# AIM-Harvard/pyradiomics

Measured on AMD Instinct MI355X. Metric: Mvoxels/s for GLCM+GLRLM build, 512^3 vol @32 bins, higher is better.
Workload: dtype u8 levels / u32 counts / f64 out; 1 GPU; GLCM+GLRLM matrix build, 512^3 int32+uint8 volume resident in HBM, 32 grey levels, full mask, 13 angles, uniform levels; one volume per GPU (batch sharding, no collective); size=512, levels=32, dist=uniform, deferred_mode=pipeline

## Files before the change

### pyradiomics_amd/csrc/kernels_sweepfw.h

```cpp
#pragma once
#include "kernels_sweep.h"

namespace prad {

enum FwPhase { FP_INIT, FP_GRAB, FP_CTRL, FP_ISSUE, FP_WAIT_ROWS, FP_WAIT_PACK, FP_GROUP, FP_PACK, FP_SLOW, FP_FLUSH, FP_DRAIN,
               FP_TOTAL, FP_REALTIME, FP_NGROUP, FP_NGROUP_PACK, FP_NSLOW, FP_COUNT };
#ifdef PRAD_FW_STAMPS
__device__ unsigned long long prad_fw_stamps[2 * 8192 * FP_COUNT];
struct FwClock {
  unsigned long long last, first, rt0;
  unsigned acc[FP_COUNT];
  __device__ __forceinline__ void start() {
#pragma unroll
    for (int i = 0; i < FP_COUNT; i++) acc[i] = 0;
    rt0 = __builtin_amdgcn_s_memrealtime();
    first = last = __builtin_readcyclecounter();
  }
  template <int PH>
  __device__ __forceinline__ void lap() {
    const unsigned long long now = __builtin_readcyclecounter();
    acc[PH] += (unsigned)(now - last);
    last = now;
  }
  template <int PH>
  __device__ __forceinline__ void count() { acc[PH]++; }
  __device__ __forceinline__ void store(int slot) {
    acc[FP_TOTAL] = (unsigned)(__builtin_readcyclecounter() - first);
    acc[FP_REALTIME] = (unsigned)(__builtin_amdgcn_s_memrealtime() - rt0);
    const unsigned w = blockIdx.x * (blockDim.x >> 6) + (threadIdx.x >> 6);
    if ((threadIdx.x & 63) == 0 && w < 8192) {
#pragma unroll
      for (int i = 0; i < FP_COUNT; i++) prad_fw_stamps[((size_t)slot * 8192 + w) * FP_COUNT + i] = acc[i];
    }
  }
};
#else
struct FwClock {
  __device__ __forceinline__ void start() {}
  template <int PH>
  __device__ __forceinline__ void lap() {}
  template <int PH>
  __device__ __forceinline__ void count() {}
  __device__ __forceinline__ void store(int) {}
};
#endif

struct FwDesc {
  int slot;
  int NM, NU;
  int du, dx;
  long long sM, sU;
  int CL, pieces;
  int chunks;
  int dom_kind;
};
struct FwSet {
  int count;
  int NX;
  int pitch;
  int nrows;
  int xcd;
  int first_block[PRAD_MAX_SWEEP + 1];
  FwDesc d[PRAD_MAX_SWEEP];
};

struct PackJob {
  const int *image;
  const uint8_t *mask;
  uint8_t *levels;
  uint8_t *levels16;
  uint8_t *rowzero;
  int *flags;
  long long n16;
  int NX, Ng;
  int every;
};

#define PRAD_FW_U 8
#ifndef PRAD_FW_MAXG
#define PRAD_FW_MAXG 4
#endif
#define PRAD_FW_WORK_STRIDE 64
#define PRAD_FW_DOMAINS 8
__host__ __device__ inline size_t fw_lds_bytes(const HistLayout &h) { return 4 * ((size_t)h.words + (size_t)(h.Ng + 1)); }


struct FwTab {
  u32 *rl_long;
  int Nr, P4, Q, lenlim, gB, RL4, RS, RL, dummy0b, alive0, deadmax;
  unsigned Qinv;
  __device__ __forceinline__ void init(const HistLayout &h, int Nr_, u32 *rl_long_) {
    rl_long = rl_long_;
    Nr = Nr_;
    Q = 4 * (h.Ng + 1);
    P4 = (h.RS + 1) * (h.Ng + 1);
    lenlim = (h.RS + 1) * Q;
    RS = h.RS;
    RL = h.RL;
    RL4 = 4 * h.RL;
    gB = Q + 4 * h.g0 - RL4 - 4 * h.RS;
    Qinv = (unsigned)((0x100000000ull + (unsigned)Q - 1) / (unsigned)Q);
    dummy0b = Q + 4 * h.dummy0;
    alive0 = (h.RS + 2) * Q;
    deadmax = (h.RS + 1) * Q;
  }
};

__device__ __noinline__ void fw_long_event(const FwTab &T, int lv, int lb) {
  const int idx = (int)__umulhi((unsigned)lb, T.Qinv);
  if (idx < T.RS + T.RL) {
    lds_bump(T.gB + __mul24(lv, T.RL4) + (idx << 2));
    return;
  }
  const unsigned key = ((unsigned)lv << 20) | (unsigned)idx;
  bool pending = true;
// ... 650 lines not shown
          row -= du * NU;
          off -= (long long)du * NU * D.sU;
          ri -= (long long)du * NU * sUr;
          zpos = 65;
          wrap = false;
          continue;
        }
        t++;
        zpos++;
        row += du;
        off += delta;
        ri += dri;
        if (du != 0 && (row < 0 || row >= NU)) wrap = true;
      }
    }
  }
};

template <bool ZA>
__device__ __forceinline__ void fw_row_word(const FwTab &T, u32 one, int &s, u32 c, u32 x) {
  int t;
#define PRAD_FW_RCOL(J)                                                                                          \
  "v_cmpx_ne_u32_sdwa vcc, %[c], %[x] src0_sel:BYTE_" #J " src1_sel:BYTE_" #J "\n\t"                             \
  "v_add_u32_sdwa %[t], %[s], %[c] dst_sel:DWORD dst_unused:UNUSED_PAD src0_sel:DWORD src1_sel:BYTE_" #J "\n\t"   \
  "v_mul_u32_u24_sdwa %[s], %[P4], %[c] dst_sel:DWORD dst_unused:UNUSED_PAD src0_sel:DWORD src1_sel:BYTE_" #J "\n\t" \
  "v_cmpx_ne_u32_sdwa vcc, %[x], %[z] src0_sel:BYTE_" #J " src1_sel:DWORD\n\t"                                  \
  "ds_add_u32 %[t], %[one]\n\t"                                                                                  \
  "s_mov_b64 exec, -1\n\t"                                                                                       \
  "v_add_u32 %[s], %[Q], %[s]\n\t"
#define PRAD_FW_RCOL_NZ(J)                                                                                       \
  "v_cmpx_ne_u32_sdwa vcc, %[c], %[x] src0_sel:BYTE_" #J " src1_sel:BYTE_" #J "\n\t"                             \
  "v_add_u32_sdwa %[t], %[s], %[c] dst_sel:DWORD dst_unused:UNUSED_PAD src0_sel:DWORD src1_sel:BYTE_" #J "\n\t"   \
  "ds_add_u32 %[t], %[one]\n\t"                                                                                  \
  "v_mul_u32_u24_sdwa %[s], %[P4], %[c] dst_sel:DWORD dst_unused:UNUSED_PAD src0_sel:DWORD src1_sel:BYTE_" #J "\n\t" \
  "s_mov_b64 exec, -1\n\t"                                                                                       \
  "v_add_u32 %[s], %[Q], %[s]\n\t"
  if (ZA) {
    u32 z = 0;
    asm volatile("" : "+v"(z));
    asm volatile(PRAD_FW_RCOL(0) PRAD_FW_RCOL(1) PRAD_FW_RCOL(2) PRAD_FW_RCOL(3)
                 : [s] "+v"(s), [t] "=&v"(t)
                 : [c] "v"(c), [x] "v"(x), [one] "v"(one), [P4] "s"(T.P4), [Q] "s"(T.Q), [z] "v"(z)
                 : "vcc", "memory");
  } else {
    asm volatile(PRAD_FW_RCOL_NZ(0) PRAD_FW_RCOL_NZ(1) PRAD_FW_RCOL_NZ(2) PRAD_FW_RCOL_NZ(3)
                 : [s] "+v"(s), [t] "=&v"(t)
                 : [c] "v"(c), [x] "v"(x), [one] "v"(one), [P4] "s"(T.P4), [Q] "s"(T.Q)
                 : "vcc", "memory");
  }
#undef PRAD_FW_RCOL
#undef PRAD_FW_RCOL_NZ
}

template <bool LONG, bool ZA>
__device__ __forceinline__ void fw_rows_role(const HistLayout &h, const FwTab &T, u32 *lds, const uint8_t *__restrict__ L,
                                             long long nrows, int NX, int pitch, int bx, int nblocks) {
  const int lane = threadIdx.x & 63, wave = threadIdx.x >> 6, wpb = blockDim.x >> 6;
  const int dummy = T.dummy0b + 4 * lane;
  u32 one = 1;
  asm volatile("" : "+v"(one));
  uint8_t *tile = reinterpret_cast<uint8_t *>(lds) + ((fw_lds_bytes(h) + 15) & ~(size_t)15) + (size_t)wave * 64 * PRAD_ROW_PITCH;
  const int RSTEP = nrows >= 4096 ? 8 : 1;
  const long long ngroups = RSTEP == 8 ? ((nrows + 511) / 512) * 8 : (nrows + 63) / 64;
  const long long nwaves = (long long)nblocks * wpb;
  const bool vec16 = (pitch & 15) == 0 && ((uintptr_t)L & 15) == 0;
  for (long long grp = (long long)bx * wpb + wave; grp < ngroups; grp += nwaves) {
    const long long r0 = RSTEP == 8 ? (grp >> 3) * 512 + (grp & 7) : grp * 64;
    int s = 0;
    u32 pw = 0;
    uint4 nx4[4];
    auto fetch = [&](int xc) __attribute__((always_inline)) {
#pragma unroll
      for (int j = 0; j < 4; j++) {
        const int rr = j * 16 + (lane >> 2);
        const int cx = xc + (lane & 3) * 16;
        uint4 q = make_uint4(0, 0, 0, 0);
        if (r0 + RSTEP * rr < nrows && cx < NX) {
          q = *reinterpret_cast<const uint4 *>(L + (r0 + RSTEP * rr) * pitch + cx);
          const int valid = NX - cx;
          if (valid < 16) {
            u32 *qw = reinterpret_cast<u32 *>(&q);
#pragma unroll
            for (int wd = 0; wd < 4; wd++) {
              const int keep = valid - 4 * wd;
              qw[wd] = keep >= 4 ? qw[wd] : (keep <= 0 ? 0u : (qw[wd] & ((1u << (8 * keep)) - 1u)));
            }
          }
        }
        nx4[j] = q;
      }
    };
    if (vec16) fetch(0);
    for (int xc = 0; xc < NX; xc += 64) {
      if (vec16) {
#pragma unroll
        for (int j = 0; j < 4; j++) *reinterpret_cast<uint4 *>(tile + (j * 16 + (lane >> 2)) * PRAD_ROW_PITCH + (lane & 3) * 16) = nx4[j];
        __builtin_amdgcn_wave_barrier();
        if (xc + 64 < NX) fetch(xc + 64);
      } else {
        const bool xin = xc + lane < NX;
#pragma unroll 8
        for (int rr = 0; rr < 64; rr++) {
          uint8_t b = 0;
          if (xin && r0 + RSTEP * rr < nrows) b = L[(r0 + RSTEP * rr) * pitch + xc + lane];
          tile[rr * PRAD_ROW_PITCH + lane] = b;
        }
      }
      __builtin_amdgcn_wave_barrier();
      const uint4 *row = reinterpret_cast<const uint4 *>(tile + lane * PRAD_ROW_PITCH);
#pragma unroll
      for (int q = 0; q < 4; q++) {
        const uint4 d = row[q];
        const u32 wds[4] = {d.x, d.y, d.z, d.w};
        const unsigned m = (pw >> 24) ? (unsigned)(s - __mul24((int)(pw >> 24), T.P4)) : 0u;
        if (LONG && __ballot(m + 16 * T.Q > (unsigned)T.lenlim) != 0) {
#pragma unroll 1
          for (int k = 0; k < 4; k++) {
            const u32 c = wds[k], x = __builtin_amdgcn_alignbyte(c, pw, 3);
            const unsigned m4 = (pw >> 24) ? (unsigned)(s - __mul24((int)(pw >> 24), T.P4)) : 0u;
            if (__ballot(m4 + 4 * T.Q > (unsigned)T.lenlim) != 0) {
#pragma unroll
              for (int b = 0; b < 4; b++) fw_checked<LONG>(T, dummy, s, (int)((x >> (8 * b)) & 0xffu), (int)((c >> (8 * b)) & 0xffu), false);
            } else {
              fw_row_word<ZA>(T, one, s, c, x);
            }
            pw = c;
          }
        } else {
#pragma unroll
          for (int k = 0; k < 4; k++) {
            fw_row_word<ZA>(T, one, s, wds[k], __builtin_amdgcn_alignbyte(wds[k], pw, 3));
            pw = wds[k];
          }
        }
      }
      __builtin_amdgcn_wave_barrier();
    }
    fw_checked<LONG>(T, dummy, s, (int)(pw >> 24), 0, false);
  }
}

template <bool LONG>
__global__ void __launch_bounds__(1024) sweep_fw_rows_kernel(const uint8_t *__restrict__ L, long long nrows, int NX, int pitch,
                                                            int slot, int Ng, int Nr, int RS, u32 *__restrict__ glcm_acc,
                                                            u32 *__restrict__ glrlm_acc, int *__restrict__ flags) {
  extern __shared__ u32 lds[];
  if (flags[0]) return;
  const HistLayout h = hist_layout(true, true, true, Ng, RS);
  if ((unsigned)(size_t)((lds_u32 *)lds) != 0u) {
    if (threadIdx.x == 0) atomicExch(flags + 2, 1);
    return;
  }
  for (int i = threadIdx.x; i < h.words + Ng + 1; i += blockDim.x) lds[i] = 0;
  __syncthreads();
  FwTab T;
  T.init(h, Nr, glrlm_acc + (size_t)slot * Ng * Nr);
  if (flags[3] != 0) fw_rows_role<LONG, true>(h, T, lds, L, nrows, NX, pitch, (int)blockIdx.x, (int)gridDim.x);
  else fw_rows_role<LONG, false>(h, T, lds, L, nrows, NX, pitch, (int)blockIdx.x, (int)gridDim.x);
  flush_block_hist<true, true, true>(lds + Ng + 1, h, Nr, slot, glcm_acc, glrlm_acc);
}

template <bool LONG, int K, bool HASPAD, bool PACK>
__global__ void __launch_bounds__(1024) sweep_fw_kernel(FwSet set, PackJob pj, const uint8_t *__restrict__ L,
                                                        const uint8_t *__restrict__ rowzero, int Ng, int Nr, int RS,
                                                        u32 *__restrict__ glcm_acc, u32 *__restrict__ glrlm_acc,
                                                        int *__restrict__ work, int *__restrict__ flags) {
  extern __shared__ u32 lds[];
  int role = 0;
  while (role + 1 < set.count && (int)blockIdx.x >= set.first_block[role + 1]) role++;
  const int bx = (int)blockIdx.x - set.first_block[role], nblocks = set.first_block[role + 1] - set.first_block[role];
  const int wpb = (int)(blockDim.x >> 6);
  const long long pw = __builtin_amdgcn_readfirstlane((int)(blockIdx.x * wpb + (threadIdx.x >> 6)));
  PackWave pk(pj, pw, (long long)gridDim.x * wpb);
  FwClock clk;
  clk.start();
#ifdef PRAD_FW_SETPRIO
  __builtin_amdgcn_s_setprio(PRAD_FW_SETPRIO);
#endif
  if (flags[0] == 0) {
    const bool anyzero = flags[3] != 0;
    const HistLayout h = hist_layout(true, true, true, Ng, RS);
    if ((unsigned)(size_t)((lds_u32 *)lds) != 0u) {
      if (threadIdx.x == 0) atomicExch(flags + 2, 1);
    } else {
      for (int i = threadIdx.x; i < h.words + Ng + 1; i += blockDim.x) lds[i] = 0;
      __syncthreads();
      clk.lap<FP_INIT>();
      const FwDesc &D = set.d[role];
      FwTab T;
      T.init(h, Nr, glrlm_acc + (size_t)D.slot * Ng * Nr);
      int *wk = work + PRAD_FW_WORK_STRIDE * PRAD_FW_DOMAINS * role;
      if (D.dx == 0) {
        FwWave<LONG, K, 0, HASPAD, PACK> w(T, set.NX);
        w.run(D, set.NX, set.pitch, set.nrows, L, rowzero, anyzero, wk, bx, nblocks, pk, pj, set.xcd != 0, clk);
      } else if (D.dx > 0) {
        FwWave<LONG, K, 1, HASPAD, PACK> w(T, set.NX);
        w.run(D, set.NX, set.pitch, set.nrows, L, rowzero, anyzero, wk, bx, nblocks, pk, pj, set.xcd != 0, clk);
      } else {
        FwWave<LONG, K, -1, HASPAD, PACK> w(T, set.NX);
        w.run(D, set.NX, set.pitch, set.nrows, L, rowzero, anyzero, wk, bx, nblocks, pk, pj, set.xcd != 0, clk);
      }
      clk.lap<FP_CTRL>();
      flush_block_hist<true, true, true>(lds + Ng + 1, h, Nr, D.slot, glcm_acc, glrlm_acc);
      clk.lap<FP_FLUSH>();
    }
  }
  if (PACK) pk.drain(pj);
  clk.lap<FP_DRAIN>();
  clk.store(PACK ? 1 : 0);
}

}
```

### pyradiomics_amd/csrc/prad_api.hip

```cpp
#include "prad_runtime.h"
#include "kernels_generic.h"
#include "kernels_pairs.h"
#include "kernels_sweep.h"
#include "kernels_sweepfw.h"
#include "kernels_sweepfw2.h"
#include "kernels_neigh.h"
#include "kernels_glszm.h"
#include "kernels_voxel.h"
#include "kernels_voxslide.h"
#include "kernels_mcc.h"
#include "kernels_voxtex.h"
#include "kernels_binning.h"

#include <algorithm>
#include <atomic>
#include <chrono>
#include <cmath>
#include <condition_variable>
#include <cstdlib>
#include <deque>
#include <limits>
#include <mutex>
#include <thread>

// ... 175 lines not shown
  Timed t(*k.c, "generic", k.s);
  hipLaunchKernelGGL(gen_gldm_kernel, dim3(blocks_for(threads)), dim3(256), 0, k.s, k.g, k.vm, k.image, k.mask,
                     k.angles_d, k.Na, Ng, alpha, out, k.flags_d + 1);
  return check_launch("gen_gldm_kernel");
}

int generic_ngtdm(Call &k, int Ng, double *out) {
  Timed t(*k.c, "generic", k.s);
  if (k.vm.voxels) {
    hipLaunchKernelGGL(gen_ngtdm_voxel_kernel, dim3(blocks_for(k.vm.nvox, 64)), dim3(64), 0, k.s, k.g, k.vm,
                       k.image, k.mask, k.angles_d, k.Na, Ng, out, k.flags_d + 1);
    return check_launch("gen_ngtdm_voxel_kernel");
  }
  unsigned long long *acc = nullptr;
  const size_t nacc = (size_t)Ng * (k.Na + 1);
  PRAD_TRY(k.c->get<unsigned long long>("ngtdm_acc", nacc, &acc));
  PRAD_HIP(hipMemsetAsync(acc, 0, sizeof(unsigned long long) * nacc, k.s));
  PRAD_TRY(check_grid(k.g.n, "NGTDM"));
  hipLaunchKernelGGL(gen_ngtdm_segment_kernel, dim3(blocks_for(k.g.n)), dim3(256), 0, k.s, k.g, k.vm, k.image,
                     k.mask, k.angles_d, k.Na, Ng, acc, k.flags_d + 1);
  PRAD_TRY(check_launch("gen_ngtdm_segment_kernel"));
  hipLaunchKernelGGL(ngtdm_finalize_kernel, dim3(blocks_for(Ng, 64)), dim3(64), 0, k.s, acc, Ng, k.Na, out);
  return check_launch("ngtdm_finalize_kernel");
}

struct SweepPlan {
  bool ok = false;
  int Nz = 1, Ny = 1, Nx = 1;
  SweepSet lines;
  int row_slot = -1;
  bool skip1 = false;
  bool fused = false;
  int LPL = 1;
  int pitch = 0, padw = 0;
  bool vec_rows = false;
  AngleSet aset;
  int RS = 0;
  bool LONG = false;
  int threads = 256;
  size_t lds_bytes = 0;
  int RSr = 0;
  bool LONGr = false;
  size_t lds_bytes_rows = 0;
  bool fw = false;
  int fwK = 8;
  int fw_blocks = 1;
  int fw_threads = 1024;
  int fw_rows_threads = 512;
  int RSfw = 0;
  bool LONGfw = false;
  size_t lds_fw = 0;
  int RSfw_rows = 0;
  size_t lds_fw_rows = 0;
  bool fw2 = false;
  int RS2 = 0;
  int fw2_copies = 1;
  bool LONGfw2 = false;
  size_t lds_fw2 = 0;
  int pitch16 = 0;
  bool fw2_rows = false;
  int RS2r = 0, fw2r_copies = 1, fw2r_waves = 16;
  bool LONGfw2r = false;
  size_t lds_fw2_rows = 0;
  FwSet fwset;
};

constexpr size_t kHistBudget = 72 * 1024;
constexpr size_t kHistBudgetRows = 36 * 1024;
constexpr int kRowsThreads = 512;
constexpr size_t kHistBudgetFw = 146 * 1024;

int cu_count() {
  static thread_local int cus = 0;
  if (!cus) {
    int dev = 0;
    if (hipGetDevice(&dev) != hipSuccess ||
        hipDeviceGetAttribute(&cus, hipDeviceAttributeMultiprocessorCount, dev) != hipSuccess || cus <= 0)
      cus = 256;
  }
  return cus;
}

int fit_rs(bool glcm, bool glrlm, bool fused, int Ng, int Nr, size_t budget) {
  int lo = 0, hi = Nr;
  if (sizeof(u32) * (size_t)hist_layout(glcm, glrlm, fused, Ng, 1).words > budget) return -1;
  lo = 1;
  while (lo < hi) {
    const int mid = (lo + hi + 1) / 2;
    if (sizeof(u32) * (size_t)hist_layout(glcm, glrlm, fused, Ng, mid).words <= budget) lo = mid;
    else hi = mid - 1;
  }
  return lo;
}

SweepPlan plan_sweep(const Call &k, int Ng, int Nr, bool want_glcm, bool want_glrlm) {
  SweepPlan p;
  if (k.vm.voxels || k.g.nd > 3 || Ng < 1 || Ng > 255 || k.Na > PRAD_MAX_SWEEP) return p;
  int dims[3] = {1, 1, 1};
  for (int d = 0; d < k.g.nd; d++) dims[3 - k.g.nd + d] = k.g.size[d];
  p.Nz = dims[0]; p.Ny = dims[1]; p.Nx = dims[2];
  const int longest = std::max(dims[0], std::max(dims[1], dims[2]));
  if (want_glrlm && Nr < longest) return p;
  if (!want_glrlm) Nr = 1;
  if (want_glcm && want_glrlm) {
    const int rs = fit_rs(true, true, true, Ng, Nr, kHistBudget);
    const int rsr = fit_rs(true, true, true, Ng, Nr, kHistBudgetRows);
// ... 111 lines not shown
    int first = 0;
    for (int d = 0; d < 3; d++) {
      if (o[d] < -1 || o[d] > 1) return p;
      if (!first && o[d]) first = o[d];
      p.aset.off[a][d] = o[d];
    }
    if (first != 1) return p;
    if (o[0] == 0 && o[1] == 0) {
      if (p.row_slot >= 0) return p;
      p.row_slot = a;
      continue;
    }
    SweepDesc &D = p.lines.d[p.lines.count++];
    D.slot = a;
    D.NX = p.Nx;
    D.dx = o[2];
    if (o[0] == 1) {
      D.NM = p.Nz; D.NU = p.Ny; D.du = o[1];
      D.sM = (long long)p.Ny * p.pitch; D.sU = p.pitch;
    } else {
      D.NM = p.Ny; D.NU = p.Nz; D.du = 0;
      D.sM = p.pitch; D.sU = (long long)p.Ny * p.pitch;
    }
    D.LXc = (p.Nx + 64 * p.LPL - 1) / (64 * p.LPL);
    D.chunks = (long long)D.NU * D.LXc;
  }
  if ((p.fw || p.fw2) && p.lines.count > 0) {
    size_t budget = kHistBudgetFw;
    if (const char *e = getenv("PRAD_FW_BUDGET_KB")) budget = (size_t)std::max(8, atoi(e)) * 1024;
    p.RSfw = fit_rs(true, true, true, Ng, Nr, budget);
    if (p.RSfw < Nr) {
      for (int rs = p.RSfw; rs >= std::max(16, p.RSfw - 12); rs--) {
        const int d = (((rs + 1) * (Ng + 1)) % 32 + 1) % 32, dist = std::min(d, 32 - d);
        if ((d & 1) && dist >= 5 && dist <= 11) {
          p.RSfw = rs;
          break;
        }
      }
    }
    if (const char *e = getenv("PRAD_FW_RS")) p.RSfw = std::max(1, std::min(p.RSfw, atoi(e)));
    p.LONGfw = p.RSfw < Nr;
    p.lds_fw = fw_lds_bytes(hist_layout(true, true, true, Ng, p.RSfw));
    if (p.row_slot >= 0 && p.fw) {
      if (const char *e = getenv("PRAD_FW_ROWS_THREADS")) p.fw_rows_threads = std::max(64, std::min(1024, atoi(e) & ~63));
      const size_t tiles = (size_t)(p.fw_rows_threads / 64) * 64 * PRAD_ROW_PITCH;
      int rs = fit_rs(true, true, true, Ng, Nr, std::min<size_t>(100 * 1024, (size_t)160 * 1024 - 2048 - tiles));
      for (int r = rs; rs < Nr && r >= std::max(16, rs - 12); r--) {
        const int d = (((r + 1) * (Ng + 1)) % 32 + 1) % 32, dist = std::min(d, 32 - d);
        if ((d & 1) && dist >= 5 && dist <= 11) { rs = r; break; }
      }
      p.RSfw_rows = rs;
      p.lds_fw_rows = ((fw_lds_bytes(hist_layout(true, true, true, Ng, rs)) + 15) & ~(size_t)15) + tiles;
    }
    {
      const int nroles = p.lines.count;
      int total = cu_count();
      if (const char *e = getenv("PRAD_FW_BLOCKS")) total = std::max(nroles, atoi(e));
      if (const char *e = getenv("PRAD_FW_THREADS")) p.fw_threads = std::max(64, std::min(1024, atoi(e) & ~63));
      int bonus[PRAD_MAX_SWEEP] = {0};
      {
        int left = total % nroles;
        const bool as_listed = getenv("PRAD_FW_EXTRA_FIRST") != nullptr;
        for (int cls = as_listed ? 0 : 2; cls >= 0 && left > 0; cls--)
          for (int r = 0; r < nroles && left > 0; r++) {
            const SweepDesc &S = p.lines.d[r];
            const int c = (S.dx != 0 ? 1 : 0) + (S.du != 0 ? 1 : 0);
            if ((as_listed || c == cls) && !bonus[r]) {
              bonus[r] = 1;
              left--;
            }
          }
      }
      p.fwset.first_block[0] = 0;
      for (int r = 0; r < nroles; r++) p.fwset.first_block[r + 1] = p.fwset.first_block[r] + total / nroles + bonus[r];
      for (int r = nroles + 1; r < PRAD_MAX_SWEEP + 1; r++) p.fwset.first_block[r] = p.fwset.first_block[nroles];
      p.fw_blocks = p.fwset.first_block[nroles];
    }
    int per_wave = 6;
    if (const char *e = getenv("PRAD_FW_PER_WAVE")) per_wave = std::max(1, atoi(e));
    p.fwset.count = p.lines.count;
    p.fwset.NX = p.Nx;
    p.fwset.xcd = 0;
    if (const char *e = getenv("PRAD_FW_XCD")) p.fwset.xcd = ((p.fw || p.fw2) && p.Nz >= 64 && atoi(e) != 0) ? 1 : 0;
    for (int i = 0; i < p.lines.count; i++) {
      const SweepDesc &S = p.lines.d[i];
      FwDesc &D = p.fwset.d[i];
      D.slot = S.slot; D.NM = S.NM; D.NU = S.NU; D.du = S.du; D.dx = S.dx; D.sM = S.sM; D.sU = S.sU;
      p.fwset.pitch = p.pitch;
      if (p.fw2) {
        const bool march_z = S.sM >= S.sU;
        D.sM = march_z ? (long long)p.Ny * p.pitch16 : p.pitch16;
        D.sU = march_z ? p.pitch16 : (long long)p.Ny * p.pitch16;
        p.fwset.pitch = p.pitch16;
      }
      p.fwset.nrows = p.Nz * p.Ny;
      const long long want = (long long)per_wave * (p.fwset.first_block[i + 1] - p.fwset.first_block[i]) * (p.fw_threads / 64);
      int pieces = (int)std::max<long long>(1, (want + D.NU - 1) / D.NU);
      int CL = ((D.NM + pieces - 1) / pieces + 7) & ~7;
      CL = std::max(CL, D.NM >= 128 ? 64 : 16);
      const bool march_z_role = S.sM >= S.sU && p.Nz > 1;
      D.dom_kind = march_z_role ? 0 : 1;
      if (p.fwset.xcd && march_z_role) CL = std::max(32, ((D.NM + PRAD_FW_DOMAINS - 1) / PRAD_FW_DOMAINS + 7) & ~7);
      if (const char *e = getenv("PRAD_FW_CL")) CL = std::max(8, atoi(e) & ~7);
      D.CL = CL;
      D.pieces = (D.NM + CL - 1) / CL;
      const long long chunks = (long long)D.NU * D.pieces;
      if (chunks > 2000000000LL) return p;
      D.chunks = (int)chunks;
    }
  } else {
    p.fw = false;
    if (p.fw2) return SweepPlan();
  }
  if (p.row_slot < 0) p.skip1 = false;
  p.ok = true;
  return p;
}

template <bool G, bool R, bool LNG, bool F, int LPL>
int launch_lines_lpl(Call &k, const SweepPlan &p, const uint8_t *levels, int Ng, int Nr, u32 *glcm_acc,
                     u32 *glrlm_acc, int *multi) {
  long long maxchunks = 0;
  for (int i = 0; i < p.lines.count; i++) maxchunks = std::max(maxchunks, p.lines.d[i].chunks);
  const int wpb = p.threads / 64;
  const long long blocks_avail = std::max<long long>(1, (long long)cu_count() / p.lines.count);
  unsigned gx = (unsigned)std::max<long long>(1, std::min<long long>(blocks_avail, (maxchunks + wpb - 1) / wpb));
  if (const char *e = getenv("PRAD_LINES_BLOCKS")) {
    const int v = atoi(e);
    if (v >= 1) gx = (unsigned)v;
  }
  PRAD_HIP(hipFuncSetAttribute(reinterpret_cast<const void *>(&sweep_lines_kernel<G, R, LNG, F, LPL>),
                               hipFuncAttributeMaxDynamicSharedMemorySize, (int)p.lds_bytes));
  hipLaunchKernelGGL((sweep_lines_kernel<G, R, LNG, F, LPL>), dim3(gx, p.lines.count), dim3(p.threads), p.lds_bytes,
                     k.s, p.lines, levels, Ng, Nr, p.RS, glcm_acc, glrlm_acc, multi, multi + PRAD_MAX_SWEEP,
                     k.flags_d);
  return check_launch("sweep_lines_kernel");
}

template <bool G, bool R, bool LNG, bool F>
int launch_lines(Call &k, const SweepPlan &p, const uint8_t *levels, int Ng, int Nr, u32 *glcm_acc, u32 *glrlm_acc,
                 int *multi) {
  if (p.LPL == 4) return launch_lines_lpl<G, R, LNG, F, 4>(k, p, levels, Ng, Nr, glcm_acc, glrlm_acc, multi);
  if (p.LPL == 2) return launch_lines_lpl<G, R, LNG, F, 2>(k, p, levels, Ng, Nr, glcm_acc, glrlm_acc, multi);
  return launch_lines_lpl<G, R, LNG, F, 1>(k, p, levels, Ng, Nr, glcm_acc, glrlm_acc, multi);
}

template <bool LNG, int K, bool HASPAD, bool PACK>
int launch_fw_kpp(Call &k, const SweepPlan &p, const PackJob &pj, const uint8_t *levels, const uint8_t *rowzero, int Ng, int Nr,
                  u32 *glcm_acc, u32 *glrlm_acc, int *multi, int *flags_d) {
  PRAD_HIP(hipFuncSetAttribute(reinterpret_cast<const void *>(&sweep_fw_kernel<LNG, K, HASPAD, PACK>),
                               hipFuncAttributeMaxDynamicSharedMemorySize, (int)p.lds_fw));
  hipLaunchKernelGGL((sweep_fw_kernel<LNG, K, HASPAD, PACK>), dim3(p.fw_blocks), dim3(p.fw_threads), p.lds_fw, k.s, p.fwset, pj,
                     levels, rowzero, Ng, Nr, p.RSfw, glcm_acc, glrlm_acc, multi + 2 * PRAD_MAX_SWEEP + PRAD_FW_WORK_STRIDE, flags_d);
  return check_launch("sweep_fw_kernel");
}
template <bool LNG, int K, bool HASPAD>
int launch_fw_kp(Call &k, const SweepPlan &p, const PackJob &pj, const uint8_t *levels, const uint8_t *rowzero, int Ng, int Nr,
                 u32 *glcm_acc, u32 *glrlm_acc, int *multi, int *flags_d) {
  if (pj.n16 > 0) return launch_fw_kpp<LNG, K, HASPAD, true>(k, p, pj, levels, rowzero, Ng, Nr, glcm_acc, glrlm_acc, multi, flags_d);
  return launch_fw_kpp<LNG, K, HASPAD, false>(k, p, pj, levels, rowzero, Ng, Nr, glcm_acc, glrlm_acc, multi, flags_d);
}
template <bool LNG, int K>
int launch_fw_k(Call &k, const SweepPlan &p, const PackJob &pj, const uint8_t *levels, const uint8_t *rowzero, int Ng, int Nr,
                u32 *glcm_acc, u32 *glrlm_acc, int *multi, int *flags_d) {
  if (p.Nx != 64 * K) return launch_fw_kp<LNG, K, true>(k, p, pj, levels, rowzero, Ng, Nr, glcm_acc, glrlm_acc, multi, flags_d);
  return launch_fw_kp<LNG, K, false>(k, p, pj, levels, rowzero, Ng, Nr, glcm_acc, glrlm_acc, multi, flags_d);
}
int launch_fw(Call &k, const SweepPlan &p, const PackJob &pj, const uint8_t *levels, const uint8_t *rowzero, int Ng, int Nr,
              u32 *glcm_acc, u32 *glrlm_acc, int *multi, int *flags_d) {
  if (p.fwK == 16)
    return p.LONGfw ? launch_fw_k<true, 16>(k, p, pj, levels, rowzero, Ng, Nr, glcm_acc, glrlm_acc, multi, flags_d)
                    : launch_fw_k<false, 16>(k, p, pj, levels, rowzero, Ng, Nr, glcm_acc, glrlm_acc, multi, flags_d);
  if (p.LONGfw) return p.fwK == 4 ? launch_fw_k<true, 4>(k, p, pj, levels, rowzero, Ng, Nr, glcm_acc, glrlm_acc, multi, flags_d)
                                : launch_fw_k<true, 8>(k, p, pj, levels, rowzero, Ng, Nr, glcm_acc, glrlm_acc, multi, flags_d);
  return p.fwK == 4 ? launch_fw_k<false, 4>(k, p, pj, levels, rowzero, Ng, Nr, glcm_acc, glrlm_acc, multi, flags_d)
                    : launch_fw_k<false, 8>(k, p, pj, levels, rowzero, Ng, Nr, glcm_acc, glrlm_acc, multi, flags_d);
}

template <bool LNG, int K, bool HASPAD, bool SKIP1, bool PACK>
int launch_fw2_khsp(Call &k, const SweepPlan &p, const PackJob &pj, const uint8_t *levels16, int Ng, int Nr, u32 *glcm_acc, u32 *glrlm_acc,
                    int *work, int *flags_d) {
  PRAD_HIP(hipFuncSetAttribute(reinterpret_cast<const void *>(&sweep_fw2_kernel<LNG, K, HASPAD, SKIP1, PACK>),
                               hipFuncAttributeMaxDynamicSharedMemorySize, (int)p.lds_fw2));
  hipLaunchKernelGGL((sweep_fw2_kernel<LNG, K, HASPAD, SKIP1, PACK>), dim3(p.fw_blocks), dim3(1024), p.lds_fw2, k.s, p.fwset, pj, levels16,
                     Ng, Nr, p.RS2, p.fw2_copies, glcm_acc, glrlm_acc, work, flags_d);
  return check_launch("sweep_fw2_kernel");
}
template <bool LNG, int K, bool HASPAD, bool SKIP1>
int launch_fw2_khs(Call &k, const SweepPlan &p, const PackJob &pj, const uint8_t *levels16, int Ng, int Nr, u32 *glcm_acc, u32 *glrlm_acc,
                   int *work, int *flags_d) {
  if (pj.n16 > 0) return launch_fw2_khsp<LNG, K, HASPAD, SKIP1, true>(k, p, pj, levels16, Ng, Nr, glcm_acc, glrlm_acc, work, flags_d);
  return launch_fw2_khsp<LNG, K, HASPAD, SKIP1, false>(k, p, pj, levels16, Ng, Nr, glcm_acc, glrlm_acc, work, flags_d);
}
template <bool LNG, int K>
int launch_fw2_k(Call &k, const SweepPlan &p, const PackJob &pj, const uint8_t *levels16, int Ng, int Nr, u32 *glcm_acc, u32 *glrlm_acc,
                 int *multi, int *flags_d) {
  int *work = multi + 2 * PRAD_MAX_SWEEP + PRAD_FW_WORK_STRIDE;
  if (p.Nx != 64 * K)
    return p.skip1 ? launch_fw2_khs<LNG, K, true, true>(k, p, pj, levels16, Ng, Nr, glcm_acc, glrlm_acc, work, flags_d)
                   : launch_fw2_khs<LNG, K, true, false>(k, p, pj, levels16, Ng, Nr, glcm_acc, glrlm_acc, work, flags_d);
  return p.skip1 ? launch_fw2_khs<LNG, K, false, true>(k, p, pj, levels16, Ng, Nr, glcm_acc, glrlm_acc, work, flags_d)
                 : launch_fw2_khs<LNG, K, false, false>(k, p, pj, levels16, Ng, Nr, glcm_acc, glrlm_acc, work, flags_d);
}
int launch_fw2(Call &k, const SweepPlan &p, const PackJob &pj, const uint8_t *levels16, int Ng, int Nr, u32 *glcm_acc, u32 *glrlm_acc,
               int *multi, int *flags_d) {
  if (p.LONGfw2) return p.fwK == 4 ? launch_fw2_k<true, 4>(k, p, pj, levels16, Ng, Nr, glcm_acc, glrlm_acc, multi, flags_d)
                                 : launch_fw2_k<true, 8>(k, p, pj, levels16, Ng, Nr, glcm_acc, glrlm_acc, multi, flags_d);
  return p.fwK == 4 ? launch_fw2_k<false, 4>(k, p, pj, levels16, Ng, Nr, glcm_acc, glrlm_acc, multi, flags_d)
                    : launch_fw2_k<false, 8>(k, p, pj, levels16, Ng, Nr, glcm_acc, glrlm_acc, multi, flags_d);
}

template <bool LNG>
int launch_fw_rows(Call &k, const SweepPlan &p, const uint8_t *levels, int Ng, int Nr, u32 *glcm_acc, u32 *glrlm_acc, int *flags_d) {
  const long long nrows = (long long)p.Nz * p.Ny, groups = nrows >= 4096 ? ((nrows + 511) / 512) * 8 : (nrows + 63) / 64;
  const int wpb = p.fw_rows_threads / 64;
  const unsigned gx = (unsigned)std::max<long long>(1, std::min<long long>((groups + wpb - 1) / wpb, (long long)cu_count()));
  PRAD_HIP(hipFuncSetAttribute(reinterpret_cast<const void *>(&sweep_fw_rows_kernel<LNG>),
                               hipFuncAttributeMaxDynamicSharedMemorySize, (int)p.lds_fw_rows));
  hipLaunchKernelGGL((sweep_fw_rows_kernel<LNG>), dim3(gx), dim3(p.fw_rows_threads), p.lds_fw_rows, k.s, levels, nrows, p.Nx,
                     p.pitch, p.row_slot, Ng, Nr, p.RSfw_rows, glcm_acc, glrlm_acc, flags_d);
  return check_launch("sweep_fw_rows_kernel");
}

template <bool LNG>
int launch_fw2_rows(Call &k, const SweepPlan &p, const uint8_t *levels16, int Ng, int Nr, u32 *glcm_acc, u32 *glrlm_acc, int *flags_d) {
  const long long nrows = (long long)p.Nz * p.Ny, groups = nrows >= 4096 ? ((nrows + 511) / 512) * 8 : (nrows + 63) / 64;
  const int wpb = p.fw2r_waves;
  const unsigned gx = (unsigned)std::max<long long>(1, std::min<long long>((groups + wpb - 1) / wpb, (long long)cu_count()));
  PRAD_HIP(hipFuncSetAttribute(reinterpret_cast<const void *>(&sweep_fw2_rows_kernel<LNG>),
                               hipFuncAttributeMaxDynamicSharedMemorySize, (int)p.lds_fw2_rows));
  hipLaunchKernelGGL((sweep_fw2_rows_kernel<LNG>), dim3(gx), dim3(64 * wpb), p.lds_fw2_rows, k.s, levels16, nrows, p.Nx, p.pitch16,
                     p.row_slot, Ng, Nr, p.RS2r, p.fw2r_copies, glcm_acc, glrlm_acc, flags_d);
  return check_launch("sweep_fw2_rows_kernel");
}

template <bool G, bool R, bool LNG, bool F>
int launch_rows(Call &k, const SweepPlan &p, const uint8_t *levels, int Ng, int Nr, u32 *glcm_acc, u32 *glrlm_acc,
                int *multi) {
  const long long nrows = (long long)p.Nz * p.Ny;
  const long long groups = (nrows + 63) / 64;
  const int wpb = kRowsThreads / 64;
  const int per_cu = std::max(1, std::min(2048 / kRowsThreads, (int)(160 * 1024 / p.lds_bytes_rows)));
  const unsigned gx = (unsigned)std::max<long long>(1, std::min<long long>((groups + wpb - 1) / wpb, (long long)cu_count() * per_cu));
  PRAD_HIP(hipFuncSetAttribute(reinterpret_cast<const void *>(&sweep_rows_kernel<G, R, LNG, F>),
                               hipFuncAttributeMaxDynamicSharedMemorySize, (int)p.lds_bytes_rows));
  hipLaunchKernelGGL((sweep_rows_kernel<G, R, LNG, F>), dim3(gx), dim3(kRowsThreads), p.lds_bytes_rows, k.s, levels,
                     nrows, p.Nx, p.pitch, p.row_slot, Ng, Nr, p.RSr, glcm_acc, glrlm_acc, multi, k.flags_d);
  return check_launch("sweep_rows_kernel");
}

__global__ void __launch_bounds__(256) zero3_kernel(u32 *__restrict__ a, size_t na, u32 *__restrict__ b, size_t nb,
                                                    u32 *__restrict__ c3, size_t nc) {
  const size_t t = (size_t)blockIdx.x * blockDim.x + threadIdx.x, nt = (size_t)gridDim.x * blockDim.x;
  uint4 *a4 = reinterpret_cast<uint4 *>(a);
  for (size_t i = t; i < na / 4; i += nt) a4[i] = make_uint4(0, 0, 0, 0);
  for (size_t i = (na & ~(size_t)3) + t; i < na; i += nt) a[i] = 0;
  for (size_t i = t; i < nb; i += nt) b[i] = 0;
  for (size_t i = t; i < nc; i += nt) c3[i] = 0;
}

struct VolState {
  bool valid = false;
  SweepPlan p;
  int Ng = 0, Nr = 0, Na = 0;
  double *glcm = nullptr, *glrlm = nullptr;
  uint8_t *levels = nullptr, *rowzero = nullptr;
  uint8_t *levels16 = nullptr;
// ... 59 lines not shown
    return false;
  if (k.g.n >= (1LL << 31)) return false;
  if (v.p.fw2) return v.levels16 && v.p.pitch16 == 2 * v.p.Nx && (((uintptr_t)v.levels16) & 15) == 0;
  return v.p.fw && v.p.fused;
}

PackJob make_pack_job(const Call &k, const VolState &v, const VolState *host) {
  PackJob j;
  memset(&j, 0, sizeof(j));
  j.image = k.image;
  j.mask = k.mask;
  j.levels = v.levels;
  j.levels16 = v.p.fw2 ? v.levels16 : nullptr;
  j.rowzero = v.rowzero;
  j.flags = v.flags_d;
  j.n16 = k.g.n / 16;
  j.NX = v.p.Nx;
  j.Ng = v.Ng;
  double groups = 0, waves = 16.0;
  if (host) {
    for (int i = 0; i < host->p.fwset.count; i++) groups += (double)host->p.fwset.d[i].NM * host->p.fwset.d[i].NU / PRAD_FW_U;
    waves = 16.0 * std::max(1, host->p.fw_blocks);
  }
  const double units = (double)j.n16 / 64.0;
  const double slack = v.p.fw2 ? 1.05 : 0.92;
  j.every = (int)std::max(1.0, std::min(64.0, std::floor(slack * groups / std::max(1.0, units))));
  (void)waves;
  if (const char *e = getenv("PRAD_PACK_EVERY")) j.every = std::max(1, atoi(e));
  return j;
}

int vol_pack_standalone(Call &k, VolState &v) {
  Context &c = *k.c;
  const SweepPlan &p = v.p;
  Timed t(c, "pack", k.s);
  if (p.fw2) {
    const unsigned gx = (unsigned)std::max<long long>(1, std::min<long long>((k.g.n / 4 + 255) / 256, 8192));
    hipLaunchKernelGGL(pack_levels16_kernel, dim3(gx), dim3(256), 0, k.s, k.image, k.mask, k.g.n, p.Nx, p.pitch16, p.pitch, v.Ng,
                       v.levels16, v.levels, v.flags_d);
    return check_launch("pack_levels16_kernel");
  }
  const int vec_ok = p.vec_rows && ((((uintptr_t)k.image) | ((uintptr_t)k.mask) | ((uintptr_t)v.levels)) & 15) == 0;
  const unsigned gx = (unsigned)std::max<long long>(1, std::min<long long>((k.g.n / 16 + 255) / 256, 4096));
  const int shift = (v.glcm && v.glrlm && p.fused) ? PRAD_FUSED_SHIFT : 0;
  hipLaunchKernelGGL(pack_levels_kernel, dim3(gx), dim3(256), 0, k.s, k.image, k.mask, k.g.n, p.Nx, p.pitch, p.padw,
                     v.Ng, v.levels, v.flags_d, vec_ok, shift, v.rowzero);
  return check_launch("pack_levels_kernel");
}

template <bool G, bool R, bool F>
int launch_sweeps(Call &k, const VolState &v, const PackJob &pj) {
  const SweepPlan &p = v.p;
  if (p.lines.count > 0 && p.fw && G && R && F) {
    static const bool rows_side = getenv("PRAD_ROWS_STREAM") != nullptr;
    if (rows_side && p.row_slot >= 0) {
      static thread_local hipStream_t side = nullptr;
      static thread_local hipEvent_t e0 = nullptr, e1 = nullptr;
      if (!side) {
        int lo = 0, hi = 0;
        PRAD_HIP(hipDeviceGetStreamPriorityRange(&lo, &hi));
        PRAD_HIP(hipStreamCreateWithPriority(&side, hipStreamNonBlocking, getenv("PRAD_ROWS_STREAM_PRIO") ? atoi(getenv("PRAD_ROWS_STREAM_PRIO")) : lo));
        PRAD_HIP(hipEventCreateWithFlags(&e0, hipEventDisableTiming));
        PRAD_HIP(hipEventCreateWithFlags(&e1, hipEventDisableTiming));
      }
      PRAD_HIP(hipEventRecord(e0, k.s));
      PRAD_HIP(hipStreamWaitEvent(side, e0, 0));
      {
        Timed t(*k.c, "sweep", k.s);
        PRAD_TRY(launch_fw(k, p, pj, v.levels, v.rowzero, v.Ng, v.Nr, v.glcm_acc, v.glrlm_acc, v.multi, v.flags_d));
      }
      Call k2 = k;
      k2.s = side;
      if (p.RSfw_rows < v.Nr) PRAD_TRY(launch_fw_rows<true>(k2, p, v.levels, v.Ng, v.Nr, v.glcm_acc, v.glrlm_acc, v.flags_d));
      else PRAD_TRY(launch_fw_rows<false>(k2, p, v.levels, v.Ng, v.Nr, v.glcm_acc, v.glrlm_acc, v.flags_d));
      PRAD_HIP(hipEventRecord(e1, side));
      PRAD_HIP(hipStreamWaitEvent(k.s, e1, 0));
      return PRAD_OK;
    }
    {
      Timed t(*k.c, "sweep", k.s);
      PRAD_TRY(launch_fw(k, p, pj, v.levels, v.rowzero, v.Ng, v.Nr, v.glcm_acc, v.glrlm_acc, v.multi, v.flags_d));
    }
    if (p.row_slot >= 0) {
      Timed t(*k.c, "rows", k.s);
      if (p.RSfw_rows < v.Nr) PRAD_TRY(launch_fw_rows<true>(k, p, v.levels, v.Ng, v.Nr, v.glcm_acc, v.glrlm_acc, v.flags_d));
      else PRAD_TRY(launch_fw_rows<false>(k, p, v.levels, v.Ng, v.Nr, v.glcm_acc, v.glrlm_acc, v.flags_d));
    }
    return PRAD_OK;
  }
  if (p.fw2 && G && R && !F && p.lines.count > 0) {
    {
      Timed t(*k.c, "sweep", k.s);
      PRAD_TRY(launch_fw2(k, p, pj, v.levels16, v.Ng, v.Nr, v.glcm_acc, v.glrlm_acc, v.multi, v.flags_d));
    }
    if (p.row_slot >= 0) {
      Timed t(*k.c, "rows", k.s);
      if (p.fw2_rows) {
        if (p.LONGfw2r) PRAD_TRY(launch_fw2_rows<true>(k, p, v.levels16, v.Ng, v.Nr, v.glcm_acc, v.glrlm_acc, v.flags_d));
        else PRAD_TRY(launch_fw2_rows<false>(k, p, v.levels16, v.Ng, v.Nr, v.glcm_acc, v.glrlm_acc, v.flags_d));
      } else if (p.LONGr) {
        PRAD_TRY((launch_rows<G, R, true, F>(k, p, v.levels, v.Ng, v.Nr, v.glcm_acc, v.glrlm_acc, v.multi)));
      } else {
        PRAD_TRY((launch_rows<G, R, false, F>(k, p, v.levels, v.Ng, v.Nr, v.glcm_acc, v.glrlm_acc, v.multi)));
      }
    }
    return PRAD_OK;
  }
  Timed t(*k.c, "sweep", k.s);
  if (p.lines.count > 0) {
    if (R && p.LONG) PRAD_TRY((launch_lines<G, R, true, F>(k, p, v.levels, v.Ng, v.Nr, v.glcm_acc, v.glrlm_acc, v.multi)));
    else PRAD_TRY((launch_lines<G, R, false, F>(k, p, v.levels, v.Ng, v.Nr, v.glcm_acc, v.glrlm_acc, v.multi)));
  }
  if (p.row_slot >= 0) {
    if (R && p.LONGr) PRAD_TRY((launch_rows<G, R, true, F>(k, p, v.levels, v.Ng, v.Nr, v.glcm_acc, v.glrlm_acc, v.multi)));
    else PRAD_TRY((launch_rows<G, R, false, F>(k, p, v.levels, v.Ng, v.Nr, v.glcm_acc, v.glrlm_acc, v.multi)));
  }
  return PRAD_OK;
}

int vol_sweep(Call &k, const VolState &v, const PackJob &pj) {
  if (pj.n16 > 0 && !pipeline_volume(v.p, v.glcm != nullptr, v.glrlm != nullptr))
    return fail(PRAD_E_ARG, "internal: a pack job needs a fixed-window host launch");
  if (pj.n16 > 0 && (pj.levels16 != nullptr) != v.p.fw2)
    return fail(PRAD_E_ARG, "internal: the pack job's layout is not the host launch's");
  if (v.glcm && v.glrlm && v.p.fused) return launch_sweeps<true, true, true>(k, v, pj);
  if (v.glcm && v.glrlm) return launch_sweeps<true, true, false>(k, v, pj);
  if (v.glcm) return launch_sweeps<true, false, false>(k, v, pj);
  return launch_sweeps<false, true, false>(k, v, pj);
}

__global__ void latch_flags_kernel(const int *__restrict__ flags, int *__restrict__ sticky) {
  if (flags[0] || flags[2]) sticky[0] = 1;
}

__global__ void latch_any_flag_kernel(const int *__restrict__ flags, int *__restrict__ sticky) {
  if (flags[0] || flags[1] || flags[2]) sticky[0] = 1;
// ... 1662 lines not shown
```

Baseline: 286,900 Mvoxels/s.

## Fold row-direction sweep into fused fw kernel as extra blocks with dynamic stealing

Removes the separate rows kernel launch and instead appends extra blocks to the fused sweep_fw kernel that process the row (x-direction) groups concurrently with the other angle roles. Row groups beyond the static first pass are handed out dynamically via per-XCC-domain atomic heads with work stealing across domains. This aims to remove the serial tail and launch gap of the rows pass and balance load. The cost is larger LDS per block (max of both layouts) and always using the LONG template for the rows path, which may lower occupancy or add checks. The PRAD_ROWS_STREAM side-stream option is also removed.

```diff
diff --git a/pyradiomics_amd/csrc/kernels_sweepfw.h b/pyradiomics_amd/csrc/kernels_sweepfw.h
--- a/pyradiomics_amd/csrc/kernels_sweepfw.h
+++ b/pyradiomics_amd/csrc/kernels_sweepfw.h
@@ -61,6 +61,10 @@
   int nrows;
   int xcd;
   int first_block[PRAD_MAX_SWEEP + 1];
+  int xslot;
+  int xRS;
+  int xwaves;
+  int xgpd;
   FwDesc d[PRAD_MAX_SWEEP];
 };
 
@@ -817,19 +821,31 @@
 #undef PRAD_FW_RCOL_NZ
 }
 
+__host__ __device__ inline long long fw_row_groups(long long nrows) {
+  return nrows >= 4096 ? ((nrows + 511) / 512) * 8 : (nrows + 63) / 64;
+}
+
 template <bool LONG, bool ZA>
 __device__ __forceinline__ void fw_rows_role(const HistLayout &h, const FwTab &T, u32 *lds, const uint8_t *__restrict__ L,
-                                             long long nrows, int NX, int pitch, int bx, int nblocks) {
-  const int lane = threadIdx.x & 63, wave = threadIdx.x >> 6, wpb = blockDim.x >> 6;
+                                             long long nrows, int NX, int pitch, int bx, int nblocks, int wave, int wpb,
+                                             int *heads, int gpd) {
+  const int lane = threadIdx.x & 63;
   const int dummy = T.dummy0b + 4 * lane;
   u32 one = 1;
   asm volatile("" : "+v"(one));
   uint8_t *tile = reinterpret_cast<uint8_t *>(lds) + ((fw_lds_bytes(h) + 15) & ~(size_t)15) + (size_t)wave * 64 * PRAD_ROW_PITCH;
   const int RSTEP = nrows >= 4096 ? 8 : 1;
-  const long long ngroups = RSTEP == 8 ? ((nrows + 511) / 512) * 8 : (nrows + 63) / 64;
+  const long long ngroups = fw_row_groups(nrows);
   const long long nwaves = (long long)nblocks * wpb;
   const bool vec16 = (pitch & 15) == 0 && ((uintptr_t)L & 15) == 0;
-  for (long long grp = (long long)bx * wpb + wave; grp < ngroups; grp += nwaves) {
+  const int ndyn = (heads && ngroups > nwaves) ? (int)(ngroups - nwaves) : 0;
+  int bnext = 0, bend = 0, dom = 0, tried = 0;
+  if (ndyn > 0) {
+    int id;
+    asm volatile("s_getreg_b32 %0, hwreg(HW_REG_XCC_ID)" : "=s"(id));
+    dom = id & (PRAD_FW_DOMAINS - 1);
+  }
+  for (long long grp = (long long)bx * wpb + wave; grp < ngroups;) {
     const long long r0 = RSTEP == 8 ? (grp >> 3) * 512 + (grp & 7) : grp * 64;
     int s = 0;
     u32 pw = 0;
@@ -902,6 +918,31 @@
       __builtin_amdgcn_wave_barrier();
     }
     fw_checked<LONG>(T, dummy, s, (int)(pw >> 24), 0, false);
+    if (!heads) {
+      grp += nwaves;
+      continue;
+    }
+    grp = ngroups;
+    if (bnext >= bend) {
+      while (tried < PRAD_FW_DOMAINS && ndyn > 0) {
+        const int lo = (int)((long long)ndyn * dom / PRAD_FW_DOMAINS), hi = (int)((long long)ndyn * (dom + 1) / PRAD_FW_DOMAINS);
+        int got = hi;
+        if (lane == 0) {
+          int *head = heads + dom * PRAD_FW_WORK_STRIDE;
+          got = lo + __hip_atomic_load(head, __ATOMIC_RELAXED, __HIP_MEMORY_SCOPE_AGENT);
+          if (got < hi) got = lo + atomicAdd(head, gpd);
+        }
+        got = __builtin_amdgcn_readfirstlane(got);
+        if (got < hi) {
+          bnext = got;
+          bend = min(got + gpd, hi);
+          break;
+        }
+        tried++;
+        dom = (dom + 1) & (PRAD_FW_DOMAINS - 1);
+      }
+    }
+    if (bnext < bend) grp = nwaves + bnext++;
   }
 }
 
@@ -920,8 +961,9 @@
   __syncthreads();
   FwTab T;
   T.init(h, Nr, glrlm_acc + (size_t)slot * Ng * Nr);
-  if (flags[3] != 0) fw_rows_role<LONG, true>(h, T, lds, L, nrows, NX, pitch, (int)blockIdx.x, (int)gridDim.x);
-  else fw_rows_role<LONG, false>(h, T, lds, L, nrows, NX, pitch, (int)blockIdx.x, (int)gridDim.x);
+  const int wave = (int)(threadIdx.x >> 6), wpb = (int)(blockDim.x >> 6);
+  if (flags[3] != 0) fw_rows_role<LONG, true>(h, T, lds, L, nrows, NX, pitch, (int)blockIdx.x, (int)gridDim.x, wave, wpb, nullptr, 0);
+  else fw_rows_role<LONG, false>(h, T, lds, L, nrows, NX, pitch, (int)blockIdx.x, (int)gridDim.x, wave, wpb, nullptr, 0);
   flush_block_hist<true, true, true>(lds + Ng + 1, h, Nr, slot, glcm_acc, glrlm_acc);
 }
 
@@ -931,12 +973,33 @@
                                                         u32 *__restrict__ glcm_acc, u32 *__restrict__ glrlm_acc,
                                                         int *__restrict__ work, int *__restrict__ flags) {
   extern __shared__ u32 lds[];
+  const int wpb = (int)(blockDim.x >> 6);
+  if ((int)blockIdx.x >= set.first_block[set.count]) {
+    const int bx = (int)blockIdx.x - set.first_block[set.count], nblocks = set.first_block[set.count + 1] - set.first_block[set.count];
+    if (flags[0] != 0 || (long long)bx * set.xwaves >= fw_row_groups(set.nrows)) return;
+    if ((unsigned)(size_t)((lds_u32 *)lds) != 0u) {
+      if (threadIdx.x == 0) atomicExch(flags + 2, 1);
+      return;
+    }
+    const HistLayout hx = hist_layout(true, true, true, Ng, set.xRS);
+    for (int i = threadIdx.x; i < hx.words + Ng + 1; i += blockDim.x) lds[i] = 0;
+    __syncthreads();
+    FwTab T;
+    T.init(hx, Nr, glrlm_acc + (size_t)set.xslot * Ng * Nr);
+    const int wave = (int)(threadIdx.x >> 6);
+    if (wave < set.xwaves) {
+      int *heads = work + PRAD_FW_WORK_STRIDE * PRAD_FW_DOMAINS * set.count;
+      if (flags[3] != 0) fw_rows_role<true, true>(hx, T, lds, L, set.nrows, set.NX, set.pitch, bx, nblocks, wave, set.xwaves, heads, set.xgpd);
+      else fw_rows_role<true, false>(hx, T, lds, L, set.nrows, set.NX, set.pitch, bx, nblocks, wave, set.xwaves, heads, set.xgpd);
+    }
+    flush_block_hist<true, true, true>(lds + Ng + 1, hx, Nr, set.xslot, glcm_acc, glrlm_acc);
+    return;
+  }
   int role = 0;
   while (role + 1 < set.count && (int)blockIdx.x >= set.first_block[role + 1]) role++;
   const int bx = (int)blockIdx.x - set.first_block[role], nblocks = set.first_block[role + 1] - set.first_block[role];
-  const int wpb = (int)(blockDim.x >> 6);
   const long long pw = __builtin_amdgcn_readfirstlane((int)(blockIdx.x * wpb + (threadIdx.x >> 6)));
-  PackWave pk(pj, pw, (long long)gridDim.x * wpb);
+  PackWave pk(pj, pw, (long long)set.first_block[set.count] * wpb);
   FwClock clk;
   clk.start();
 #ifdef PRAD_FW_SETPRIO
diff --git a/pyradiomics_amd/csrc/prad_api.hip b/pyradiomics_amd/csrc/prad_api.hip
--- a/pyradiomics_amd/csrc/prad_api.hip
+++ b/pyradiomics_amd/csrc/prad_api.hip
@@ -251,6 +251,7 @@
   size_t lds_fw = 0;
   int RSfw_rows = 0;
   size_t lds_fw_rows = 0;
+  int fw_xblocks = 0;
   bool fw2 = false;
   int RS2 = 0;
   int fw2_copies = 1;
@@ -468,8 +469,10 @@
       p.RSfw_rows = rs;
       p.lds_fw_rows = ((fw_lds_bytes(hist_layout(true, true, true, Ng, rs)) + 15) & ~(size_t)15) + tiles;
     }
+    int nroles_x = 0;
     {
       const int nroles = p.lines.count;
+      nroles_x = nroles;
       int total = cu_count();
       if (const char *e = getenv("PRAD_FW_BLOCKS")) total = std::max(nroles, atoi(e));
       if (const char *e = getenv("PRAD_FW_THREADS")) p.fw_threads = std::max(64, std::min(1024, atoi(e) & ~63));
@@ -491,6 +494,26 @@
       for (int r = 0; r < nroles; r++) p.fwset.first_block[r + 1] = p.fwset.first_block[r] + total / nroles + bonus[r];
       for (int r = nroles + 1; r < PRAD_MAX_SWEEP + 1; r++) p.fwset.first_block[r] = p.fwset.first_block[nroles];
       p.fw_blocks = p.fwset.first_block[nroles];
+    }
+    p.fwset.xslot = -1;
+    p.fwset.xRS = 0;
+    p.fwset.xwaves = 0;
+    p.fwset.xgpd = 1;
+    {
+      const char *e = getenv("PRAD_FW_XROLE");
+      if (p.fw && p.fused && p.row_slot >= 0 && p.fw_threads == 1024 && !(e && atoi(e) == 0)) {
+        const long long groups = fw_row_groups((long long)p.Nz * p.Ny);
+        const int wpb = p.fw_rows_threads / 64;
+        long long xb = std::min<long long>((groups + wpb - 1) / wpb, (long long)cu_count());
+        if (const char *b = getenv("PRAD_FW_XBLOCKS")) xb = std::min<long long>(atoll(b), 4096);
+        p.fw_xblocks = (int)std::max<long long>(1, xb);
+        p.fwset.first_block[nroles_x + 1] = p.fw_blocks + p.fw_xblocks;
+        p.fwset.xslot = p.row_slot;
+        p.fwset.xRS = p.RSfw_rows;
+        p.fwset.xwaves = wpb;
+        p.fwset.xgpd = 1;
+        if (const char *g = getenv("PRAD_FW_XGPD")) p.fwset.xgpd = std::max(1, std::min(64, atoi(g)));
+      }
     }
     int per_wave = 6;
     if (const char *e = getenv("PRAD_FW_PER_WAVE")) per_wave = std::max(1, atoi(e));
@@ -564,9 +587,10 @@
 template <bool LNG, int K, bool HASPAD, bool PACK>
 int launch_fw_kpp(Call &k, const SweepPlan &p, const PackJob &pj, const uint8_t *levels, const uint8_t *rowzero, int Ng, int Nr,
                   u32 *glcm_acc, u32 *glrlm_acc, int *multi, int *flags_d) {
+  const size_t lds = p.fw_xblocks > 0 ? std::max(p.lds_fw, p.lds_fw_rows) : p.lds_fw;
   PRAD_HIP(hipFuncSetAttribute(reinterpret_cast<const void *>(&sweep_fw_kernel<LNG, K, HASPAD, PACK>),
-                               hipFuncAttributeMaxDynamicSharedMemorySize, (int)p.lds_fw));
-  hipLaunchKernelGGL((sweep_fw_kernel<LNG, K, HASPAD, PACK>), dim3(p.fw_blocks), dim3(p.fw_threads), p.lds_fw, k.s, p.fwset, pj,
+                               hipFuncAttributeMaxDynamicSharedMemorySize, (int)lds));
+  hipLaunchKernelGGL((sweep_fw_kernel<LNG, K, HASPAD, PACK>), dim3(p.fw_blocks + p.fw_xblocks), dim3(p.fw_threads), lds, k.s, p.fwset, pj,
                      levels, rowzero, Ng, Nr, p.RSfw, glcm_acc, glrlm_acc, multi + 2 * PRAD_MAX_SWEEP + PRAD_FW_WORK_STRIDE, flags_d);
   return check_launch("sweep_fw_kernel");
 }
@@ -628,7 +652,7 @@
 
 template <bool LNG>
 int launch_fw_rows(Call &k, const SweepPlan &p, const uint8_t *levels, int Ng, int Nr, u32 *glcm_acc, u32 *glrlm_acc, int *flags_d) {
-  const long long nrows = (long long)p.Nz * p.Ny, groups = nrows >= 4096 ? ((nrows + 511) / 512) * 8 : (nrows + 63) / 64;
+  const long long nrows = (long long)p.Nz * p.Ny, groups = fw_row_groups(nrows);
   const int wpb = p.fw_rows_threads / 64;
   const unsigned gx = (unsigned)std::max<long long>(1, std::min<long long>((groups + wpb - 1) / wpb, (long long)cu_count()));
   PRAD_HIP(hipFuncSetAttribute(reinterpret_cast<const void *>(&sweep_fw_rows_kernel<LNG>),
@@ -794,36 +818,11 @@
 int launch_sweeps(Call &k, const VolState &v, const PackJob &pj) {
   const SweepPlan &p = v.p;
   if (p.lines.count > 0 && p.fw && G && R && F) {
-    static const bool rows_side = getenv("PRAD_ROWS_STREAM") != nullptr;
-    if (rows_side && p.row_slot >= 0) {
-      static thread_local hipStream_t side = nullptr;
-      static thread_local hipEvent_t e0 = nullptr, e1 = nullptr;
-      if (!side) {
-        int lo = 0, hi = 0;
-        PRAD_HIP(hipDeviceGetStreamPriorityRange(&lo, &hi));
-        PRAD_HIP(hipStreamCreateWithPriority(&side, hipStreamNonBlocking, getenv("PRAD_ROWS_STREAM_PRIO") ? atoi(getenv("PRAD_ROWS_STREAM_PRIO")) : lo));
-        PRAD_HIP(hipEventCreateWithFlags(&e0, hipEventDisableTiming));
-        PRAD_HIP(hipEventCreateWithFlags(&e1, hipEventDisableTiming));
-      }
-      PRAD_HIP(hipEventRecord(e0, k.s));
-      PRAD_HIP(hipStreamWaitEvent(side, e0, 0));
-      {
-        Timed t(*k.c, "sweep", k.s);
-        PRAD_TRY(launch_fw(k, p, pj, v.levels, v.rowzero, v.Ng, v.Nr, v.glcm_acc, v.glrlm_acc, v.multi, v.flags_d));
-      }
-      Call k2 = k;
-      k2.s = side;
-      if (p.RSfw_rows < v.Nr) PRAD_TRY(launch_fw_rows<true>(k2, p, v.levels, v.Ng, v.Nr, v.glcm_acc, v.glrlm_acc, v.flags_d));
-      else PRAD_TRY(launch_fw_rows<false>(k2, p, v.levels, v.Ng, v.Nr, v.glcm_acc, v.glrlm_acc, v.flags_d));
-      PRAD_HIP(hipEventRecord(e1, side));
-      PRAD_HIP(hipStreamWaitEvent(k.s, e1, 0));
-      return PRAD_OK;
-    }
     {
       Timed t(*k.c, "sweep", k.s);
       PRAD_TRY(launch_fw(k, p, pj, v.levels, v.rowzero, v.Ng, v.Nr, v.glcm_acc, v.glrlm_acc, v.multi, v.flags_d));
     }
-    if (p.row_slot >= 0) {
+    if (p.row_slot >= 0 && p.fw_xblocks == 0) {
       Timed t(*k.c, "rows", k.s);
       if (p.RSfw_rows < v.Nr) PRAD_TRY(launch_fw_rows<true>(k, p, v.levels, v.Ng, v.Nr, v.glcm_acc, v.glrlm_acc, v.flags_d));
       else PRAD_TRY(launch_fw_rows<false>(k, p, v.levels, v.Ng, v.Nr, v.glcm_acc, v.glrlm_acc, v.flags_d));
```

After: 291,900 Mvoxels/s, median of 6. 1.02x the previous value.
